# phuang1024/Starst3r

Measured on AMD Instinct MI355X. Metric: 3DGS train iters/sec @ 1M Gaussians, 8x1080p views, higher is better.
Workload: dtype f32

## Files before the change

### include/st3r.h

```cpp
#ifndef ST3R_H
#define ST3R_H

#include <stdint.h>

#ifdef __cplusplus
extern "C" {
#endif

#define ST3R_VERSION 100

#define ST3R_OK 0
#define ST3R_ERR_INVALID (-1)
#define ST3R_ERR_HIP (-2)
#define ST3R_ERR_CAPACITY (-3)
#define ST3R_ERR_NOMEM (-4)
#define ST3R_ERR_PEER (-5)

#define ST3R_SPLAT_STRIDE 12
#define ST3R_MAX_VIEWS 256
#define ST3R_GRAD_PER_GAUSSIAN 23

typedef struct st3r_ctx st3r_ctx;

int st3r_version(void);
// ... 11 lines not shown
int st3r_ctx_release_scratch(st3r_ctx* ctx);
int st3r_ctx_get_stage_ms(st3r_ctx* ctx, double* ms_out, int64_t* counts_out);
const char* st3r_stage_name(int stage);


int st3r_gs_project_sh(st3r_ctx* ctx, void* stream, int N, int C, const float* means, const float* quats,
                       const float* scales, const float* opacities, const float* sh, int sh_stride,
                       const float* viewmats, const float* Ks, const float* campos, int width, int height,
                       int tile_size, float eps2d, float near_plane, float far_plane, float radius_clip,
                       float* splats, int32_t* tiles_per_gauss, double* reg_sums);

int st3r_gs_isect_scan(st3r_ctx* ctx, void* stream, int64_t n_pairs, const int32_t* tiles_per_gauss,
                       int32_t* cum_tiles, int64_t* n_isects_host);

int st3r_gs_isect_emit(st3r_ctx* ctx, void* stream, int N, int C, const float* splats,
                       const int32_t* cum_tiles, int tile_size, int tile_w, int tile_h, int64_t n_isects,
                       int64_t* isect_ids, int32_t* flatten_ids);

int st3r_gs_sort(st3r_ctx* ctx, void* stream, int64_t n_isects, int end_bit, int64_t* isect_ids,
                 int32_t* flatten_ids, int64_t* isect_ids_sorted, int32_t* flatten_ids_sorted);

int st3r_radix_sort_pairs(st3r_ctx* ctx, void* stream, int key_bytes, int64_t n, int begin_bit, int end_bit,
                          const void* keys_in, const int32_t* vals_in, void* keys_out, int32_t* vals_out);

int st3r_gs_offsets(st3r_ctx* ctx, void* stream, int64_t n_isects, const int64_t* isect_ids_sorted, int C,
                    int tile_w, int tile_h, int32_t* offsets);

int st3r_gs_blend_fwd(st3r_ctx* ctx, void* stream, int C, int width, int height, int tile_size, int tile_w,
                      int tile_h, const float* splats, const int32_t* offsets, const int32_t* flatten_ids,
                      int64_t n_isects, float* rgb, float* alpha, int32_t* last_ids);

int st3r_gs_blend_bwd(st3r_ctx* ctx, void* stream, int C, int width, int height, int tile_size, int tile_w,
                      int tile_h, const float* splats, const int32_t* offsets, const int32_t* flatten_ids,
                      int64_t n_isects, const float* alpha, const int32_t* last_ids, const float* v_rgb,
                      const float* v_alpha, const int32_t* cum_tiles, int64_t n_pairs, float* v_splats);

int st3r_gs_project_sh_bwd(st3r_ctx* ctx, void* stream, int N, int C, const float* means, const float* quats,
                           const float* scales, const float* opacities, const float* sh, int sh_stride,
                           const float* viewmats, const float* Ks, const float* campos, int width, int height,
                           float eps2d, const float* splats, const float* v_splats, float reg_views,
                           float opac_fac, float scale_fac, float* grads);

int st3r_gs_viewmat_bwd(st3r_ctx* ctx, void* stream, int N, int C, const float* means, const float* quats,
                        const float* scales, const float* sh, int sh_stride, const float* viewmats, const float* Ks,
                        const float* campos, int width, int height, float eps2d, const float* splats,
                        const float* v_splats, float* v_viewmats);
// ... 141 lines not shown
```

### starst3r_amd/_lib.py

```python
import ctypes as C
import os

_HERE = os.path.dirname(os.path.abspath(__file__))
LIB_PATH = os.path.join(_HERE, "libst3r_hip.so")

_lib = None

vp, i32, i64, f32, f64 = C.c_void_p, C.c_int, C.c_int64, C.c_float, C.c_double
u32, u64 = C.c_uint32, C.c_uint64

SIGNATURES = {
    "st3r_version": [],
    "st3r_last_error": [],
    "st3r_ctx_create": [i32, C.POINTER(vp)],
    "st3r_ctx_destroy": [vp],
    "st3r_ctx_arena_bytes": [vp],
    "st3r_ctx_peek": [vp, vp, i32, vp, i64],
    "st3r_ctx_set_profiling": [vp, i32],
    "st3r_ctx_set_debug": [vp, i32],
    "st3r_ctx_settle": [vp],
    "st3r_ctx_release_scratch": [vp],
    "st3r_ctx_get_stage_ms": [vp, C.POINTER(f64), C.POINTER(i64)],
    "st3r_stage_name": [i32],
    "st3r_gs_project_sh": [vp, vp, i32, i32, vp, vp, vp, vp, vp, i32, vp, vp, vp, i32, i32, i32, f32, f32, f32, f32,
                           vp, vp, vp],
    "st3r_gs_isect_scan": [vp, vp, i64, vp, vp, C.POINTER(i64)],
    "st3r_gs_isect_emit": [vp, vp, i32, i32, vp, vp, i32, i32, i32, i64, vp, vp],
    "st3r_gs_sort": [vp, vp, i64, i32, vp, vp, vp, vp],
    "st3r_radix_sort_pairs": [vp, vp, i32, i64, i32, i32, vp, vp, vp, vp],
    "st3r_gs_offsets": [vp, vp, i64, vp, i32, i32, i32, vp],
    "st3r_gs_blend_fwd": [vp, vp, i32, i32, i32, i32, i32, i32, vp, vp, vp, i64, vp, vp, vp],
    "st3r_gs_blend_bwd": [vp, vp, i32, i32, i32, i32, i32, i32, vp, vp, vp, i64, vp, vp, vp, vp, vp, i64, vp],
    "st3r_gs_project_sh_bwd": [vp, vp, i32, i32, vp, vp, vp, vp, vp, i32, vp, vp, vp, i32, i32, f32, vp, vp, f32, f32,
                               f32, vp],
    "st3r_gs_viewmat_bwd": [vp, vp, i32, i32, vp, vp, vp, vp, i32, vp, vp, vp, i32, i32, f32, vp, vp, vp],
    "st3r_gs_blend_depth_fwd": [vp, vp, i32, i32, i32, i32, i32, i32, vp, vp, vp, i64, vp, vp, vp],
    "st3r_gs_blend_depth_bwd": [vp, vp, i32, i32, i32, i32, i32, i32, vp, vp, vp, i64, vp, vp, vp, vp, i64, vp],
    "st3r_gs_depth_bwd": [vp, vp, i32, i32, vp, vp, vp, vp, vp, vp],
    "st3r_loss_l1_ssim": [vp, vp, i32, i32, i32, vp, vp, f32, f32, vp, vp],
    "st3r_loss_gt_moments": [vp, vp, i32, i32, i32, vp, vp],
    "st3r_ctx_set_gt_moments": [vp, vp, vp, i32, i32, i32],
    "st3r_adam_step": [vp, vp, i32, vp, vp, vp, vp, vp, i32, vp, vp, vp, f64, f64, f64, f64, i32],
    "st3r_adam_step_range": [vp, vp, i32, vp, vp, vp, vp, vp, i32, vp, vp, vp, f64, f64, f64, f64, i32, i64, i64, vp],
    "st3r_params_from_stage": [vp, vp, i32, vp, vp, vp, vp, vp, i32, vp, i64, i64, i64],
    "st3r_gs_train_fwd_bwd": [vp, vp, i32, i32, vp, vp, vp, vp, vp, i32, vp, vp, vp, vp, i32, i32, f32, f32, f32, vp,
                              vp, C.POINTER(i64)],
    "st3r_align_run": [vp, vp, i32, i32, i32, vp, vp, vp, vp, vp, vp, vp, vp, vp, vp, i32, vp, vp, vp, i32, vp, vp,
                       vp, vp, i32, vp, vp, vp, vp, i32, i32, vp, f32, i32, f32, i32, f32, vp, vp, vp, vp, vp, vp, i64,
                       vp, vp, vp],
    "st3r_align_run_opts": [vp, vp, i32, i32, i32, vp, vp, vp, vp, vp, vp, vp, vp, vp, vp, i32, vp, vp, vp, i32, vp, vp,
                            vp, vp, i32, vp, vp, vp, vp, i32, i32, vp, f32, i32, f32, i32, f32, vp, vp, vp, vp, vp, vp,
                            i64, vp, vp, vp, vp, f32, f32, f32, i32, vp, vp, vp, i64],
# ... 66 lines not shown
```

### starst3r_amd/csrc/api.hip

```cpp
#include <stdarg.h>

#include "common.h"

static thread_local char g_err[512] = "";

void st3r_set_error(const char* fmt, ...) {
    va_list ap;
    va_start(ap, fmt);
    vsnprintf(g_err, sizeof(g_err), fmt, ap);
    va_end(ap);
}

ST3R_EXPORT int st3r_version(void) { return ST3R_VERSION; }
ST3R_EXPORT const char* st3r_last_error(void) { return g_err; }

ST3R_EXPORT int st3r_ctx_create(int device, st3r_ctx** out) {
    ARG_CHECK(out);
    int ndev = 0;
    HIP_TRY(hipGetDeviceCount(&ndev));
    ARG_CHECK(device >= 0 && device < ndev);
    HIP_TRY(hipSetDevice(device));
    st3r_ctx* c = new (std::nothrow) st3r_ctx();
    if (!c) { st3r_set_error("out of host memory"); return ST3R_ERR_NOMEM; }
    memset(c, 0, sizeof(*c));
// ... 136 lines not shown
        ctx->prof_ms[st] = 0; ctx->prof_n[st] = 0;
    }
    return ST3R_OK;
}

int st3r_isect_scan_impl(st3r_ctx* ctx, hipStream_t s, int64_t n_pairs, const int32_t* tiles, int32_t* cum,
                         int64_t* n_isects_host, const void* pack_rects, int rect32, uint64_t* pack_out,
                         int32_t** total_dev_out, int32_t* total_copy, int32_t* total_host);
int st3r_isect_emit_impl(hipStream_t s, int N, int C, const float* splats, const int32_t* cum, int tile_size,
                         int tile_w, int tile_h, int64_t* isect_ids, int32_t* flatten_ids);
int st3r_sort_impl(st3r_ctx* ctx, hipStream_t s, int64_t n, int end_bit, int64_t* keys_in, int32_t* vals_in,
                   int64_t* keys_out, int32_t* vals_out);
int st3r_isect_offsets_impl(hipStream_t s, int64_t n_isects, const int64_t* ids, int C, int tile_w, int tile_h,
                            int32_t* offsets);
int st3r_project_impl(st3r_ctx* ctx, hipStream_t s, int N, int C, const float* means, const float* quats, const float* scales,
                      const float* opacities, const float* sh, int sh_stride, const float* viewmats, const float* Ks,
                      const float* campos, int width, int height, int tile_size, float eps2d, float near_plane,
                      float far_plane, float radius_clip, float* splats, int32_t* tiles_per_gauss, double* reg_sums,
                      uint64_t* depth_keys, int32_t* depth_vals, int tight, uint32_t key_base, void* rects, int rect32,
                      int reg_overwrite, double* zero_ptr, int zero_n, uint32_t* krange);
int st3r_sort_depth_seg_impl(st3r_ctx* ctx, hipStream_t s, int64_t N, int C, uint32_t* keys_in, int32_t* vals_in,
                             uint32_t* keys_out, int32_t* vals_out, const uint32_t* krange);
int st3r_isect_emit_chain_impl(st3r_ctx* ctx, hipStream_t s, int N, int C, const int32_t* perm, const void* rects,
                               int rect32, int tile_w, int tile_h, uint32_t* tile_keys, int32_t* vals, int64_t cap);
int st3r_records_prepare_impl(hipStream_t s, int N, int C, const float* splats, int tile_size, int tile_w, int tile_h,
                              int tight, int32_t* tiles, uint64_t* depth_keys, int32_t* depth_vals, uint32_t key_base,
                              void* rects, int rect32);
int st3r_isect_offsets32_impl(hipStream_t s, int64_t n_isects, const uint32_t* keys, int C, int tile_w, int tile_h,
                              int32_t* offsets, const int32_t* n_dev);
int st3r_sort_depth_impl(st3r_ctx* ctx, hipStream_t s, int64_t n, int end_bit, uint64_t* keys_in, int32_t* vals_in,
                         uint64_t* keys_out, int32_t* vals_out);
int st3r_sort_depth32_impl(st3r_ctx* ctx, hipStream_t s, int64_t n, int end_bit, uint32_t* keys_in, int32_t* vals_in,
                           uint32_t* keys_out, int32_t* vals_out);
int st3r_sort_tile_impl(st3r_ctx* ctx, hipStream_t s, int64_t n, int end_bit, uint32_t* keys_in, int32_t* vals_in,
                        uint32_t* keys_out, int32_t* vals_out, const int32_t* n_dev);
int st3r_blend_fwd_impl(st3r_ctx* ctx, hipStream_t s, int C, int W, int H, int tile_w, int tile_h,
                        const float* splats, const int32_t* offsets, const int32_t* flat, int64_t n_isects,
                        float* rgb, float* alpha, int32_t* last_ids, bool for_backward, bool end_in_offsets);
int st3r_blend_bwd_impl(st3r_ctx* ctx, hipStream_t s, int C, int W, int H, int tile_w, int tile_h,
                        const float* splats, const int32_t* offsets, const int32_t* flat, int64_t n_isects,
                        const float* alpha, const int32_t* last_ids, const float* v_rgb, const float* v_alpha,
                        const int32_t* cum, const uint64_t* rects, const uint64_t* rectbase, int tight, int64_t n_pairs,
                        float* v_splats,
                        bool end_in_offsets, st3r_vtile_ref* defer);
int st3r_project_sh_bwd_impl(hipStream_t s, int N, int C, const float* means, const float* quats, const float* scales,
                             const float* opacities, const float* sh, int sh_stride, const float* viewmats,
                             const float* Ks, const float* campos, int width, int height, float eps2d,
                             const float* splats, const float* v_splats, float reg_views, float opac_fac,
                             float scale_fac, float* grads, bool accumulate, int g_begin, int g_end, bool range_major,
                             const st3r_vtile_ref* slots);
int st3r_loss_impl(st3r_ctx* ctx, hipStream_t s, int C, int H, int W, const float* render, const float* gt,
                   float w_l1, float w_ssim, double* sums, float* v_render, bool sums_cleared);
int st3r_gather_vtile_impl(hipStream_t s, int64_t n_pairs, const st3r_vtile_ref* slots, float* v_splats);

static int bit_length_u32(uint32_t v) { int n = 0; while (v) { ++n; v >>= 1; } return n; }

static int settle_pending_count(st3r_ctx* ctx) {
    if (!ctx->count_pending) return ST3R_OK;
// ... 127 lines not shown
    st3r_prof_end(ctx, s, STG_SCAN);
    if (rc) return rc;
    if (async) {
        if (!ctx->count_event) HIP_TRY(hipEventCreateWithFlags(&ctx->count_event, hipEventDisableTiming));
        HIP_TRY(hipEventRecord(ctx->count_event, s));
        n_isects = ctx->isect_hint + ctx->isect_hint / 4 + 1024;
        if (ctx->debug_flags & 8) n_isects = ctx->isect_hint / 2;
        if (n_isects > 2147483647LL) n_isects = 2147483647LL;
        ctx->count_pending = 1; ctx->count_cap = n_isects;
        o->n_visible = -1; o->n_isects_ref = -1;
    } else {
        HIP_TRY(hipMemcpyAsync(ctx->pinned, total_dev, sizeof(int32_t), hipMemcpyDeviceToHost, s));
        if (reg_sums) HIP_TRY(hipMemcpyAsync(ctx->pinned + 1, reg_sums + 2, 2 * sizeof(double), hipMemcpyDeviceToHost, s));
        HIP_TRY(hipStreamSynchronize(s));
        n_isects = (int64_t)((int32_t*)ctx->pinned)[0];
        if (n_isects < 0) {
            st3r_set_error("more than 2^31 tile intersections in one call: split the views over more calls / GPUs");
            return ST3R_SPLIT_VIEWS;
        }
        o->n_visible = reg_sums ? (int64_t)((double*)ctx->pinned)[1] : -1;
        o->n_isects_ref = reg_sums ? (int64_t)((double*)ctx->pinned)[2] : n_isects;
        if (allow_async) { ctx->isect_hint = n_isects; ctx->hint_sig = sig; }
    }
    GET(SLOT_KEYS_A, uint32_t, n_isects, tkeys_a);
    GET(SLOT_KEYS_B, uint32_t, n_isects, tkeys_b);
    GET(SLOT_VALS_A, int32_t, n_isects, vals_a);
    GET(SLOT_VALS_B, int32_t, n_isects, vals_b);
    n_dev = total_dev;
    o->n_records = async ? -1 : n_isects;
    if (n_isects > 0) {
        st3r_prof_begin(ctx, s, STG_EMIT);
        rc = st3r_isect_emit_chain_impl(ctx, s, N, C, perm, rects, rect32, tile_w, tile_h, tkeys_a, vals_a, n_isects);
        st3r_prof_end(ctx, s, STG_EMIT);
        if (rc) return rc;
        const int end_bit = bit_length_u32((uint32_t)((int64_t)C * tile_w * tile_h - 1));
        st3r_prof_begin(ctx, s, STG_SORT);
        rc = st3r_sort_tile_impl(ctx, s, n_isects, end_bit, tkeys_a, vals_a, tkeys_b, vals_b, n_dev);
        st3r_prof_end(ctx, s, STG_SORT);
        if (rc) return rc;
    }
    st3r_prof_begin(ctx, s, STG_OFFSETS);
    rc = st3r_isect_offsets32_impl(s, n_isects, tkeys_b, C, tile_w, tile_h, offsets, n_dev);
    st3r_prof_end(ctx, s, STG_OFFSETS);
    if (rc) return rc;
    o->splats = splats; o->offsets = offsets; o->flat = vals_b; o->cum = cum; o->rects = rect32 ? nullptr : rects;
    o->rectbase = rectbase;
    o->n_isects = n_isects;
    o->tile_w = tile_w; o->tile_h = tile_h;
    return ST3R_OK;
}

__global__ void k_finalize_loss(int C, const double* __restrict__ sums, const double* __restrict__ reg_sums,
                                double inv_px, double inv_cnt, double w_l1, double w_ssim, double reg_views,
                                double opac_k, double scale_k, float* __restrict__ loss_out) {
    if (threadIdx.x == 0 && blockIdx.x == 0) {
        double loss = 0;
        for (int c = 0; c < C; ++c) loss += w_l1 * sums[2 * c] * inv_px + w_ssim * (1.0 - sums[2 * c + 1] * inv_cnt);
        loss += reg_views * (opac_k * reg_sums[0] + scale_k * reg_sums[1]);
        loss_out[0] = (float)loss;
    }
}

static int train_views(st3r_ctx* ctx, hipStream_t s, int N, int C, const float* means, const float* quats,
                       const float* scales, const float* opacities, const float* sh, int sh_stride,
                       const float* viewmats, const float* Ks, const float* campos, const float* gt_images, int W, int H,
// ... 204 lines not shown
```

### starst3r_amd/csrc/gs_isect.hip

```cpp
#include "common.h"
#include "tile_rect.h"

#define SCAN_THREADS 256
#define SCAN_ITEMS 16
#define SCAN_TILE (SCAN_THREADS * SCAN_ITEMS)

__device__ __forceinline__ int wave_incl_scan(int v) {
    const int lane = threadIdx.x & 63;
#pragma unroll
    for (int off = 1; off < 64; off <<= 1) {
        int t = __shfl_up(v, off);
        if (lane >= off) v += t;
    }
    return v;
}

__device__ __forceinline__ int block_incl_scan(int v, int* total) {
    __shared__ int wsum[4];
    const int lane = threadIdx.x & 63, w = threadIdx.x >> 6;
    int inc = wave_incl_scan(v);
    if (lane == 63) wsum[w] = inc;
    __syncthreads();
    int base = 0;
#pragma unroll
// ... 255 lines not shown
}

int st3r_isect_offsets_impl(hipStream_t s, int64_t n_isects, const int64_t* ids, int C, int tile_w, int tile_h,
                            int32_t* offsets) {
    int n_tiles = tile_w * tile_h;
    if (n_isects == 0) {
        HIP_TRY(hipMemsetAsync(offsets, 0, sizeof(int32_t) * (size_t)C * n_tiles, s));
        return ST3R_OK;
    }
    int tile_n_bits = bit_length_u32((uint32_t)n_tiles);
    hipLaunchKernelGGL(k_isect_offsets, dim3(ceil_div(n_isects, 256)), dim3(256), 0, s, n_isects, ids, C, n_tiles,
                       tile_n_bits, offsets);
    LAUNCH_CHECK();
    return ST3R_OK;
}

ST3R_EXPORT int st3r_gs_offsets(st3r_ctx* ctx, void* stream, int64_t n_isects, const int64_t* isect_ids_sorted,
                                int C, int tile_w, int tile_h, int32_t* offsets) {
    ARG_CHECK(ctx && n_isects >= 0 && C > 0 && tile_w > 0 && tile_h > 0 && offsets);
    ARG_CHECK(n_isects == 0 || isect_ids_sorted);
    return st3r_isect_offsets_impl((hipStream_t)stream, n_isects, isect_ids_sorted, C, tile_w, tile_h, offsets);
}

__global__ __launch_bounds__(256) void k_isect_offsets32(int64_t n_isects, const uint32_t* __restrict__ keys,
                                                         int64_t total, int32_t* __restrict__ offsets,
                                                         const int32_t* __restrict__ n_dev) {
    if (n_dev) n_isects = min(n_isects, (int64_t)max(*n_dev, 0));
    const int64_t tid = (int64_t)blockIdx.x * blockDim.x + threadIdx.x;
    if (n_isects == 0) {
        for (int64_t i = tid; i <= total; i += (int64_t)gridDim.x * blockDim.x) offsets[i] = 0;
        return;
    }
    const int64_t i0 = tid * 4;
    if (i0 >= n_isects) return;
    uint32_t k[4];
    if (i0 + 4 <= n_isects) {
        const uint4 v = *reinterpret_cast<const uint4*>(keys + i0);
        k[0] = v.x; k[1] = v.y; k[2] = v.z; k[3] = v.w;
    } else {
#pragma unroll
        for (int j = 0; j < 4; ++j) k[j] = i0 + j < n_isects ? keys[i0 + j] : 0u;
    }
    int64_t prev = i0 == 0 ? -1 : (int64_t)keys[i0 - 1];
#pragma unroll
    for (int j = 0; j < 4; ++j) {
        const int64_t idx = i0 + j;
        if (idx < n_isects) {
            const int64_t cur = k[j];
            for (int64_t i = prev + 1; i <= cur; ++i) offsets[i] = (int32_t)idx;
            prev = cur;
            if (idx == n_isects - 1)
                for (int64_t i = cur + 1; i <= total; ++i) offsets[i] = (int32_t)n_isects;
        }
    }
}

int st3r_isect_offsets32_impl(hipStream_t s, int64_t n_isects, const uint32_t* keys, int C, int tile_w, int tile_h,
                              int32_t* offsets, const int32_t* n_dev) {
    const int64_t total = (int64_t)C * tile_w * tile_h;
    if (n_isects == 0 && !n_dev) {
        HIP_TRY(hipMemsetAsync(offsets, 0, sizeof(int32_t) * (size_t)(total + 1), s));
        return ST3R_OK;
    }
    hipLaunchKernelGGL(k_isect_offsets32, dim3(ceil_div(n_isects > 0 ? (n_isects + 3) / 4 : 1, 256)), dim3(256), 0, s, n_isects,
                       keys, total, offsets, n_dev);
    LAUNCH_CHECK();
    return ST3R_OK;
}

__global__ __launch_bounds__(256) void k_records_prepare(int N, int64_t n_pairs, const float4* __restrict__ splats,
                                                         int tile_size, int tile_w, int tile_h, int tight,
                                                         int32_t* __restrict__ tiles, uint64_t* __restrict__ depth_keys,
                                                         int32_t* __restrict__ depth_vals, uint32_t key_base,
                                                         void* __restrict__ rects, int rect32) {
    const int64_t pid = (int64_t)blockIdx.x * blockDim.x + threadIdx.x;
    if (pid >= n_pairs) return;
    const float4 r2 = splats[pid * 3 + 2];
    const int radius = __float_as_int(r2.z);
    int ntiles = 0;
    TileRect tr = {0, 0, 0, 0};
    if (radius > 0) {
        const float4 r0 = splats[pid * 3 + 0];
        tr = ref_tile_rect(r0.x, r0.y, (float)radius, tile_size, tile_w, tile_h);
        if (tight) {
            const float4 r1 = splats[pid * 3 + 1];
            tr = tight_tile_rect(tr, r0.x, r0.y, r0.z, r0.w, r1.x, r1.y);
        }
        ntiles = (tr.y1 - tr.y0) * (tr.x1 - tr.x0);
// ... 70 lines not shown
__global__ __launch_bounds__(1024) void k_isect_wg_scan(int n, const int32_t* __restrict__ wg_tiles,
                                                        long long* __restrict__ wg_base) {
    __shared__ long long s_wave[16];
    const int t = threadIdx.x, lane = t & 63, w = t >> 6;
    const int per = (n + 1023) / 1024;
    const int e0 = min(t * per, n), e1 = min(e0 + per, n);
    long long sum = 0;
    for (int e = e0; e < e1; ++e) sum += wg_tiles[e];
    long long inc = sum;
#pragma unroll
    for (int off = 1; off < 64; off <<= 1) {
        const long long o = __shfl_up(inc, off);
        if (lane >= off) inc += o;
    }
    if (lane == 63) s_wave[w] = inc;
    __syncthreads();
    long long base = 0;
#pragma unroll
    for (int i = 0; i < 16; ++i) base += i < w ? s_wave[i] : 0;
    long long run = base + inc - sum;
    for (int e = e0; e < e1; ++e) { wg_base[e] = run; run += wg_tiles[e]; }
}

__global__ __launch_bounds__(256) void k_isect_emit_d(int N, int C, int bpc, const int32_t* __restrict__ perm,
                                                      const void* __restrict__ rects_d, int rect32,
                                                      const long long* __restrict__ wg_base,
                                                      const int32_t* __restrict__ wg_tiles, int tile_w, int tile_h,
                                                      uint32_t* __restrict__ tile_keys, int32_t* __restrict__ vals,
                                                      int64_t cap) {
    __shared__ int s_end[EP];
    __shared__ uint32_t s_org[EP];
    __shared__ uint16_t s_w[EP];
    __shared__ int32_t s_pid[EP];
    __shared__ uint16_t s_own[ECH];
    __shared__ unsigned s_wmax[4];
    __shared__ long long s_bsum[4];
    int c, k;
    emit_item(C, bpc, &c, &k);
    const int t = threadIdx.x, lane = t & 63, w = t >> 6;
    long long bsum = 0;
    if (!wg_base) {
        const int nb4 = (c * bpc + k) >> 2;
        for (int i = t; i < nb4; i += 256) {
            const int4 v = reinterpret_cast<const int4*>(wg_tiles)[i];
            bsum += ((long long)v.x + v.y) + ((long long)v.z + v.w);
        }
        if (t < ((c * bpc + k) & 3)) bsum += wg_tiles[4 * nb4 + t];
    }
    const int64_t first = (int64_t)c * N + (int64_t)k * EP;
    const int np = (int)min((int64_t)EP, (int64_t)(c + 1) * N - first);
    int cnt[EPT];
// ... 68 lines not shown
            if (ww < w) pre = max(pre, s_wmax[ww]);
        carry_owner = (int)max(max(max((unsigned)carry_owner, s_wmax[0]), max(s_wmax[1], s_wmax[2])), s_wmax[3]);
#pragma unroll
        for (int i = 0; i < 8; ++i) {
            const unsigned lo = max(wv[i] & 0xFFFFu, pre), hi = max(wv[i] >> 16, pre);
            wv[i] = lo | (hi << 16);
        }
        reinterpret_cast<uint4*>(s_own)[2 * t] = make_uint4(wv[0], wv[1], wv[2], wv[3]);
        reinterpret_cast<uint4*>(s_own)[2 * t + 1] = make_uint4(wv[4], wv[5], wv[6], wv[7]);
        __syncthreads();
        const int lim = min(ECH, total - c0);
        for (int i = t; i < lim; i += 256) {
            const int p = (int)s_own[i] - 1;
            const int o = c0 + i;
            const int kk = o - (p == 0 ? 0 : s_end[p - 1]);
            const uint32_t w_ = s_w[p], org = s_org[p];
            int qq = (int)((float)kk * __builtin_amdgcn_rcpf((float)w_));
            int rem = kk - qq * (int)w_;
            if (rem < 0) { --qq; rem += (int)w_; }
            if (rem >= (int)w_) { ++qq; rem -= (int)w_; }
            const uint32_t tx = (org & 0xFFFF) + (uint32_t)rem, ty = (org >> 16) + (uint32_t)qq;
            const long long pos = base + o;
            if (pos >= 0 && pos < cap) {
                tile_keys[pos] = key0 + ty * (uint32_t)tile_w + tx;
                vals[pos] = s_pid[p];
            }
        }
        __syncthreads();
    }
}

int st3r_isect_emit_chain_impl(st3r_ctx* ctx, hipStream_t s, int N, int C, const int32_t* perm, const void* rects,
                               int rect32, int tile_w, int tile_h, uint32_t* tile_keys, int32_t* vals, int64_t cap) {
    const int64_t n_pairs = (int64_t)N * C;
    if (n_pairs == 0) return ST3R_OK;
    const int bpc = ceil_div(N, EP);
    const int grid = C * bpc;
    void* p;
    int rc = st3r_arena_get(ctx, SLOT_RECTS_D, (rect32 ? sizeof(uint32_t) : sizeof(uint64_t)) * (size_t)n_pairs, &p);
    if (rc) return rc;
    void* rects_d = p;
    rc = st3r_arena_get(ctx, SLOT_CUM_D, (sizeof(long long) + sizeof(int32_t)) * (size_t)grid + 16, &p);
    if (rc) return rc;
    long long* wg_base = (long long*)p;
    int32_t* wg_tiles = (int32_t*)(wg_base + grid);
    if (((uintptr_t)wg_tiles & 15) != 0) wg_tiles += 2;
    hipLaunchKernelGGL(k_isect_gather, dim3(grid), dim3(256), 0, s, N, C, bpc, perm, rects, rect32, rects_d, wg_tiles);
    const bool self_base = grid <= EMIT_SELF_BASE_MAX;
    if (!self_base) hipLaunchKernelGGL(k_isect_wg_scan, dim3(1), dim3(1024), 0, s, grid, wg_tiles, wg_base);
    hipLaunchKernelGGL(k_isect_emit_d, dim3(grid), dim3(256), 0, s, N, C, bpc, perm, rects_d, rect32,
                       self_base ? (const long long*)nullptr : wg_base, wg_tiles, tile_w, tile_h, tile_keys, vals, cap);
    LAUNCH_CHECK();
    return ST3R_OK;
}
```

### starst3r_amd/csrc/gs_sort.hip

```cpp
#include "common.h"
#include "radix_sort.h"

int st3r_sort_impl(st3r_ctx* ctx, hipStream_t s, int64_t n, int end_bit, int64_t* keys_in, int32_t* vals_in,
                   int64_t* keys_out, int32_t* vals_out) {
    if (end_bit > 64) end_bit = 64;
    return st3r_radix_sort_u64(ctx, s, n, 0, end_bit, reinterpret_cast<const uint64_t*>(keys_in), vals_in,
                               reinterpret_cast<uint64_t*>(keys_out), vals_out);
}

int st3r_sort_depth_impl(st3r_ctx* ctx, hipStream_t s, int64_t n, int end_bit, uint64_t* keys_in, int32_t* vals_in,
                         uint64_t* keys_out, int32_t* vals_out) {
    return st3r_radix_sort_u64(ctx, s, n, 0, end_bit, keys_in, vals_in, keys_out, vals_out);
}

int st3r_sort_depth32_impl(st3r_ctx* ctx, hipStream_t s, int64_t n, int end_bit, uint32_t* keys_in, int32_t* vals_in,
                           uint32_t* keys_out, int32_t* vals_out) {
    return st3r_radix_sort_u32(ctx, s, n, 0, end_bit, keys_in, vals_in, keys_out, vals_out);
}

int st3r_sort_depth_seg_impl(st3r_ctx* ctx, hipStream_t s, int64_t N, int C, uint32_t* keys_in, int32_t* vals_in,
                             uint32_t* keys_out, int32_t* vals_out, const uint32_t* krange) {
    return st3r_radix_sort_u32_segments(ctx, s, N, C, keys_in, vals_in, keys_out, vals_out, krange);
}

int st3r_sort_tile_impl(st3r_ctx* ctx, hipStream_t s, int64_t n, int end_bit, uint32_t* keys_in, int32_t* vals_in,
                        uint32_t* keys_out, int32_t* vals_out, const int32_t* n_dev) {
    if (n_dev) return st3r_radix_sort_u32_devcount(ctx, s, n, n_dev, 0, end_bit, keys_in, vals_in, keys_out, vals_out);
    return st3r_radix_sort_u32(ctx, s, n, 0, end_bit, keys_in, vals_in, keys_out, vals_out);
}

ST3R_EXPORT int st3r_gs_sort(st3r_ctx* ctx, void* stream, int64_t n_isects, int end_bit, int64_t* isect_ids,
                             int32_t* flatten_ids, int64_t* isect_ids_sorted, int32_t* flatten_ids_sorted) {
    ARG_CHECK(ctx && n_isects >= 0 && end_bit > 0);
    if (n_isects == 0) return ST3R_OK;
    ARG_CHECK(isect_ids && flatten_ids && isect_ids_sorted && flatten_ids_sorted);
    return st3r_sort_impl(ctx, (hipStream_t)stream, n_isects, end_bit, isect_ids, flatten_ids, isect_ids_sorted,
                          flatten_ids_sorted);
}

ST3R_EXPORT int st3r_radix_sort_pairs(st3r_ctx* ctx, void* stream, int key_bytes, int64_t n, int begin_bit, int end_bit,
                                      const void* keys_in, const int32_t* vals_in, void* keys_out, int32_t* vals_out) {
    ARG_CHECK(ctx && n >= 0 && (key_bytes == 4 || key_bytes == 8) && begin_bit >= 0 && end_bit > begin_bit);
    ARG_CHECK(end_bit <= 8 * key_bytes && n < 2147483647LL);
    if (n == 0) return ST3R_OK;
    ARG_CHECK(keys_in && keys_out && ((vals_in == nullptr) == (vals_out == nullptr)));
    if (key_bytes == 4)
        return st3r_radix_sort_u32(ctx, (hipStream_t)stream, n, begin_bit, end_bit, (const uint32_t*)keys_in, vals_in,
                                   (uint32_t*)keys_out, vals_out);
    return st3r_radix_sort_u64(ctx, (hipStream_t)stream, n, begin_bit, end_bit, (const uint64_t*)keys_in, vals_in,
                               (uint64_t*)keys_out, vals_out);
}
```

### starst3r_amd/csrc/radix_sort.h

```cpp
#pragma once
#include "common.h"

int st3r_radix_sort_u32(st3r_ctx* ctx, hipStream_t s, int64_t n, int begin_bit, int end_bit, const uint32_t* keys_in,
                        const int32_t* vals_in, uint32_t* keys_out, int32_t* vals_out);
int st3r_radix_sort_u64(st3r_ctx* ctx, hipStream_t s, int64_t n, int begin_bit, int end_bit, const uint64_t* keys_in,
                        const int32_t* vals_in, uint64_t* keys_out, int32_t* vals_out);
int st3r_radix_sort_u32_devcount(st3r_ctx* ctx, hipStream_t s, int64_t n_cap, const int32_t* n_dev, int begin_bit,
                                 int end_bit, const uint32_t* keys_in, const int32_t* vals_in, uint32_t* keys_out,
                                 int32_t* vals_out);
int st3r_radix_sort_u32_segments(st3r_ctx* ctx, hipStream_t s, int64_t seg_n, int n_seg, const uint32_t* keys_in,
                                 const int32_t* vals_in, uint32_t* keys_out, int32_t* vals_out, const uint32_t* krange);
```

### starst3r_amd/csrc/radix_sort.hip

```cpp
#include "radix_sort.h"

namespace {

constexpr int RB = 8;
constexpr int RADIX = 1 << RB;
#ifndef RS_THREADS
#define RS_THREADS 1024
#endif
#ifndef RS_SMALL_BELOW
#define RS_SMALL_BELOW 100
#endif
constexpr int THREADS_L = RS_THREADS, THREADS_S = 512;
constexpr int HIST_THREADS = 256;
constexpr int HIST_ITEMS = 16;
constexpr int MAX_PASSES = 8;
constexpr int HIST_COPIES = 8;

typedef unsigned long long u64;
constexpr u64 FLAG_AGG = 1ull << 62, FLAG_INC = 2ull << 62, VALUE_MASK = (1ull << 62) - 1;

template <typename K> struct Traits;
#ifndef RS_IPT32
#define RS_IPT32 16
#endif
template <> struct Traits<uint32_t> { static constexpr int IPT = RS_IPT32, IPT_S = 8; };
template <> struct Traits<uint64_t> { static constexpr int IPT = 8, IPT_S = 4; };

__device__ __forceinline__ int wave_incl_scan_u32(uint32_t v, int lane) {
#pragma unroll
    for (int off = 1; off < 64; off <<= 1) {
        const uint32_t t = __shfl_up(v, off);
        if (lane >= off) v += t;
    }
    return v;
}

__device__ __forceinline__ uint32_t pair_lane_u32(uint32_t v, int q) {
    return q == 0 ? (uint32_t)__builtin_amdgcn_mov_dpp((int)v, 0xA0, 0xf, 0xf, true)
                  : (uint32_t)__builtin_amdgcn_mov_dpp((int)v, 0xF5, 0xf, 0xf, true);
}
__device__ __forceinline__ uint32_t quad_lane_u32(uint32_t v, int q) {
    switch (q) {
        case 0: return (uint32_t)__builtin_amdgcn_mov_dpp((int)v, 0x00, 0xf, 0xf, true);
        case 1: return (uint32_t)__builtin_amdgcn_mov_dpp((int)v, 0x55, 0xf, 0xf, true);
        case 2: return (uint32_t)__builtin_amdgcn_mov_dpp((int)v, 0xAA, 0xf, 0xf, true);
        default: return (uint32_t)__builtin_amdgcn_mov_dpp((int)v, 0xFF, 0xf, 0xf, true);
    }
}

template <typename K>
__global__ __launch_bounds__(HIST_THREADS) void k_rs_hist(const K* __restrict__ keys, int64_t n, int begin_bit,
                                                          int end_bit, int passes, uint32_t* __restrict__ hist,
                                                          const int32_t* __restrict__ n_dev) {
    __shared__ uint32_t sh[HIST_THREADS / 64][MAX_PASSES * RADIX];
    if (n_dev) n = min(n, (int64_t)max(*n_dev, 0));
    for (int i = threadIdx.x; i < (HIST_THREADS / 64) * MAX_PASSES * RADIX; i += HIST_THREADS) (&sh[0][0])[i] = 0;
    __syncthreads();
    uint32_t* mine = sh[threadIdx.x >> 6];
    constexpr int CH = HIST_THREADS * HIST_ITEMS;
    for (int64_t base = (int64_t)blockIdx.x * CH; base < n; base += (int64_t)gridDim.x * CH) {
        K k[HIST_ITEMS];
#pragma unroll
        for (int i = 0; i < HIST_ITEMS; ++i) {
            const int64_t idx = base + i * HIST_THREADS + threadIdx.x;
            k[i] = idx < n ? keys[idx] : K(0);
        }
#pragma unroll
        for (int i = 0; i < HIST_ITEMS; ++i) {
            if (base + i * HIST_THREADS + threadIdx.x < n) {
                for (int p = 0; p < passes; ++p) {
                    const int shift = begin_bit + RB * p;
                    const int bits = min(RB, end_bit - shift);
                    atomicAdd(&mine[p * RADIX + ((uint32_t)(k[i] >> shift) & ((1u << bits) - 1u))], 1u);
                }
            }
        }
    }
    __syncthreads();
    for (int i = threadIdx.x; i < passes * RADIX; i += HIST_THREADS) {
        uint32_t t = 0;
#pragma unroll
        for (int w = 0; w < HIST_THREADS / 64; ++w) t += sh[w][i];
// ... 224 lines not shown
    __syncthreads();
#pragma unroll
    for (int i = 0; i < IPT; ++i) {
        const int p = i * THREADS + tid;
        if (p < tcount) {
            const K k = sbuf[p];
            const uint32_t d = (uint32_t)(k >> shift) & dmask;
            const long long o = gofs[d] + p;
            if (!(SEG && last_seg_pass)) kout[o] = k;
            if (has_vals) vout[o] = svals[p];
        }
    }
}

inline size_t align256(size_t v) { return (v + 255) & ~(size_t)255; }

template <typename K>
int sort_pairs(st3r_ctx* ctx, hipStream_t s, int64_t n, int begin_bit, int end_bit, const K* keys_in,
               const int32_t* vals_in, K* keys_out, int32_t* vals_out, const int32_t* n_dev = nullptr) {
    if (n == 0) return ST3R_OK;
    if (end_bit > (int)sizeof(K) * 8) end_bit = (int)sizeof(K) * 8;
    if (begin_bit < 0 || begin_bit >= end_bit) { st3r_set_error("radix sort: empty bit range"); return ST3R_ERR_INVALID; }
    const int passes = (end_bit - begin_bit + RB - 1) / RB;
    constexpr int TILE_L = THREADS_L * Traits<K>::IPT, TILE_S = THREADS_S * Traits<K>::IPT_S;
    const bool small = (n + TILE_L - 1) / TILE_L < RS_SMALL_BELOW;
    const int64_t TILE = small ? TILE_S : TILE_L;
    const int64_t ntiles = (n + TILE - 1) / TILE;
    const size_t hist_bytes = align256(sizeof(uint32_t) * (size_t)(HIST_COPIES * MAX_PASSES * RADIX + MAX_PASSES));
    const size_t status_bytes = sizeof(u64) * (size_t)passes * (size_t)ntiles * RADIX;
    const size_t meta_bytes = hist_bytes + align256(status_bytes);
    const bool need_tmp = passes > 1;
    const size_t tk_bytes = need_tmp ? align256(sizeof(K) * (size_t)n) : 0;
    const size_t tv_bytes = need_tmp && vals_in ? align256(sizeof(int32_t) * (size_t)n) : 0;
    void* p;
    int rc = st3r_arena_get(ctx, SLOT_SORT_TMP, meta_bytes + tk_bytes + tv_bytes, &p);
    if (rc) return rc;
    char* base = (char*)p;
    uint32_t* hist = (uint32_t*)base;
    uint32_t* counters = hist + HIST_COPIES * MAX_PASSES * RADIX;
    u64* status = (u64*)(base + hist_bytes);
    K* tk = (K*)(base + meta_bytes);
    int32_t* tv = (int32_t*)(base + meta_bytes + tk_bytes);
    HIP_TRY(hipMemsetAsync(base, 0, meta_bytes, s));
    const int hist_blocks = (int)min((int64_t)1024, (n + HIST_THREADS * HIST_ITEMS - 1) / (HIST_THREADS * HIST_ITEMS));
    hipLaunchKernelGGL(k_rs_hist<K>, dim3(hist_blocks), dim3(HIST_THREADS), 0, s, keys_in, n, begin_bit, end_bit, passes,
                       hist, n_dev);
    const K* kin = keys_in;
    const int32_t* vin = vals_in;
    for (int ps = 0; ps < passes; ++ps) {
        const bool to_out = ((passes - 1 - ps) & 1) == 0;
        K* ko = to_out ? keys_out : tk;
        int32_t* vo = to_out ? vals_out : tv;
        const int shift = begin_bit + RB * ps;
        const int bits = min(RB, end_bit - shift);
        if (small)
            hipLaunchKernelGGL((k_rs_pass<K, THREADS_S, Traits<K>::IPT_S>), dim3((unsigned)ntiles), dim3(THREADS_S), 0, s, kin,
                               vin, ko, vin ? vo : nullptr, n, shift, bits, hist + ps * RADIX,
                               status + (size_t)ps * ntiles * RADIX, counters + ps, n_dev);
        else
            hipLaunchKernelGGL((k_rs_pass<K, THREADS_L, Traits<K>::IPT>), dim3((unsigned)ntiles), dim3(THREADS_L), 0, s, kin,
                               vin, ko, vin ? vo : nullptr, n, shift, bits, hist + ps * RADIX,
                               status + (size_t)ps * ntiles * RADIX, counters + ps, n_dev);
        kin = ko;
        if (vin) vin = vo;
    }
    LAUNCH_CHECK();
    return ST3R_OK;
}

// ... 42 lines not shown

}

int st3r_radix_sort_u32_segments(st3r_ctx* ctx, hipStream_t s, int64_t seg_n, int n_seg, const uint32_t* keys_in,
                                 const int32_t* vals_in, uint32_t* keys_out, int32_t* vals_out, const uint32_t* krange) {
    return sort_pairs_seg(ctx, s, seg_n, n_seg, keys_in, vals_in, keys_out, vals_out, krange);
}

int st3r_radix_sort_u32(st3r_ctx* ctx, hipStream_t s, int64_t n, int begin_bit, int end_bit, const uint32_t* keys_in,
                        const int32_t* vals_in, uint32_t* keys_out, int32_t* vals_out) {
    return sort_pairs<uint32_t>(ctx, s, n, begin_bit, end_bit, keys_in, vals_in, keys_out, vals_out);
}

int st3r_radix_sort_u64(st3r_ctx* ctx, hipStream_t s, int64_t n, int begin_bit, int end_bit, const uint64_t* keys_in,
                        const int32_t* vals_in, uint64_t* keys_out, int32_t* vals_out) {
    return sort_pairs<uint64_t>(ctx, s, n, begin_bit, end_bit, keys_in, vals_in, keys_out, vals_out);
}

int st3r_radix_sort_u32_devcount(st3r_ctx* ctx, hipStream_t s, int64_t n_cap, const int32_t* n_dev, int begin_bit,
                                 int end_bit, const uint32_t* keys_in, const int32_t* vals_in, uint32_t* keys_out,
                                 int32_t* vals_out) {
    return sort_pairs<uint32_t>(ctx, s, n_cap, begin_bit, end_bit, keys_in, vals_in, keys_out, vals_out, n_dev);
}
```

### starst3r_amd/ops.py

```python
import ctypes as C
import math

import torch

from . import _lib

SPLAT = 12
TILE = 16


class Context:

    def __init__(self, device):
        self.device = torch.device(device)
        if self.device.type != "cuda":
            raise _lib.St3rError(f"the st3r hot path needs a GPU device, got {device!r} (no CPU fallback)")
        idx = self.device.index if self.device.index is not None else torch.cuda.current_device()
        self.device = torch.device("cuda", idx)
        self._h = C.c_void_p()
        with torch.cuda.device(idx):
            _lib.check(_lib.lib().st3r_ctx_create(idx, C.byref(self._h)))
        import os
        if os.environ.get("ST3R_DEBUG_FLAGS"):
            _lib.check(_lib.lib().st3r_ctx_set_debug(self._h, int(os.environ["ST3R_DEBUG_FLAGS"])))
# ... 91 lines not shown

def isect(ctx, splats, tiles, N, Cn, W, H):
    tw, th = tile_grid(W, H)
    cum = torch.empty_like(tiles)
    n = C.c_int64(0)
    _lib.check(_lib.lib().st3r_gs_isect_scan(ctx.handle, _stream(), N * Cn, _p(tiles, torch.int32),
                                             _p(cum, torch.int32), C.byref(n)))
    n = n.value
    ids = torch.empty((n,), dtype=torch.int64, device=splats.device)
    flat = torch.empty((n,), dtype=torch.int32, device=splats.device)
    _lib.check(_lib.lib().st3r_gs_isect_emit(ctx.handle, _stream(), N, Cn, _p(splats), _p(cum, torch.int32), TILE, tw,
                                             th, n, _p(ids, torch.int64), _p(flat, torch.int32)))
    return cum, ids, flat


def radix_sort_pairs(ctx, keys, vals, begin_bit, end_bit):
    assert keys.dtype in (torch.int32, torch.int64)
    kb = 4 if keys.dtype == torch.int32 else 8
    ko = torch.empty_like(keys)
    vo = torch.empty_like(vals) if vals is not None else None
    _lib.check(_lib.lib().st3r_radix_sort_pairs(ctx.handle, _stream(), kb, keys.numel(), begin_bit, end_bit,
                                                _p(keys, keys.dtype), _p(vals, torch.int32), _p(ko, keys.dtype),
                                                _p(vo, torch.int32)))
    return ko, vo


def sort_pairs(ctx, ids, flat, end_bit):
    ids_in, flat_in = ids.clone(), flat.clone()
    ids_out, flat_out = torch.empty_like(ids), torch.empty_like(flat)
    _lib.check(_lib.lib().st3r_gs_sort(ctx.handle, _stream(), ids.numel(), end_bit, _p(ids_in, torch.int64),
                                       _p(flat_in, torch.int32), _p(ids_out, torch.int64),
                                       _p(flat_out, torch.int32)))
    return ids_out, flat_out


def offsets(ctx, ids_sorted, Cn, W, H):
    tw, th = tile_grid(W, H)
    off = torch.empty((Cn, th, tw), dtype=torch.int32, device=ids_sorted.device)
    _lib.check(_lib.lib().st3r_gs_offsets(ctx.handle, _stream(), ids_sorted.numel(), _p(ids_sorted, torch.int64), Cn,
                                          tw, th, _p(off, torch.int32)))
    return off


def blend_fwd(ctx, splats, off, flat, Cn, W, H):
    tw, th = tile_grid(W, H)
    dev = splats.device
# ... 359 lines not shown
```

Before: 190.7.

## Use 16-bit tile keys for intersection emit, sort and offsets when they fit

When the total tile count across views fits in 16 bits, tile keys are stored as uint16. The emit, radix sort (including a paired histogram read) and offsets kernels are templated on key width to work with them. This halves key memory traffic and arena footprint in the sort pipeline. It adds template instantiations, a new exported u16 sort, and a fallback to 32-bit keys via a debug flag or when the tile count is large.

```diff
diff --git a/include/st3r.h b/include/st3r.h
--- a/include/st3r.h
+++ b/include/st3r.h
@@ -57,6 +57,9 @@
 
 int st3r_radix_sort_pairs(st3r_ctx* ctx, void* stream, int key_bytes, int64_t n, int begin_bit, int end_bit,
                           const void* keys_in, const int32_t* vals_in, void* keys_out, int32_t* vals_out);
+
+int st3r_radix_sort_u16(st3r_ctx* ctx, void* stream, int64_t n, int begin_bit, int end_bit, const uint16_t* keys_in,
+                        const int32_t* vals_in, uint16_t* keys_out, int32_t* vals_out);
 
 int st3r_gs_offsets(st3r_ctx* ctx, void* stream, int64_t n_isects, const int64_t* isect_ids_sorted, int C,
                     int tile_w, int tile_h, int32_t* offsets);
diff --git a/starst3r_amd/_lib.py b/starst3r_amd/_lib.py
--- a/starst3r_amd/_lib.py
+++ b/starst3r_amd/_lib.py
@@ -28,6 +28,7 @@
     "st3r_gs_isect_emit": [vp, vp, i32, i32, vp, vp, i32, i32, i32, i64, vp, vp],
     "st3r_gs_sort": [vp, vp, i64, i32, vp, vp, vp, vp],
     "st3r_radix_sort_pairs": [vp, vp, i32, i64, i32, i32, vp, vp, vp, vp],
+    "st3r_radix_sort_u16": [vp, vp, i64, i32, i32, vp, vp, vp, vp],
     "st3r_gs_offsets": [vp, vp, i64, vp, i32, i32, i32, vp],
     "st3r_gs_blend_fwd": [vp, vp, i32, i32, i32, i32, i32, i32, vp, vp, vp, i64, vp, vp, vp],
     "st3r_gs_blend_bwd": [vp, vp, i32, i32, i32, i32, i32, i32, vp, vp, vp, i64, vp, vp, vp, vp, vp, i64, vp],
diff --git a/starst3r_amd/csrc/api.hip b/starst3r_amd/csrc/api.hip
--- a/starst3r_amd/csrc/api.hip
+++ b/starst3r_amd/csrc/api.hip
@@ -182,18 +182,19 @@
 int st3r_sort_depth_seg_impl(st3r_ctx* ctx, hipStream_t s, int64_t N, int C, uint32_t* keys_in, int32_t* vals_in,
                              uint32_t* keys_out, int32_t* vals_out, const uint32_t* krange);
 int st3r_isect_emit_chain_impl(st3r_ctx* ctx, hipStream_t s, int N, int C, const int32_t* perm, const void* rects,
-                               int rect32, int tile_w, int tile_h, uint32_t* tile_keys, int32_t* vals, int64_t cap);
+                               int rect32, int tile_w, int tile_h, void* tile_keys, int key16, int32_t* vals,
+                               int64_t cap);
 int st3r_records_prepare_impl(hipStream_t s, int N, int C, const float* splats, int tile_size, int tile_w, int tile_h,
                               int tight, int32_t* tiles, uint64_t* depth_keys, int32_t* depth_vals, uint32_t key_base,
                               void* rects, int rect32);
-int st3r_isect_offsets32_impl(hipStream_t s, int64_t n_isects, const uint32_t* keys, int C, int tile_w, int tile_h,
+int st3r_isect_offsets32_impl(hipStream_t s, int64_t n_isects, const void* keys, int key16, int C, int tile_w, int tile_h,
                               int32_t* offsets, const int32_t* n_dev);
 int st3r_sort_depth_impl(st3r_ctx* ctx, hipStream_t s, int64_t n, int end_bit, uint64_t* keys_in, int32_t* vals_in,
                          uint64_t* keys_out, int32_t* vals_out);
 int st3r_sort_depth32_impl(st3r_ctx* ctx, hipStream_t s, int64_t n, int end_bit, uint32_t* keys_in, int32_t* vals_in,
                            uint32_t* keys_out, int32_t* vals_out);
-int st3r_sort_tile_impl(st3r_ctx* ctx, hipStream_t s, int64_t n, int end_bit, uint32_t* keys_in, int32_t* vals_in,
-                        uint32_t* keys_out, int32_t* vals_out, const int32_t* n_dev);
+int st3r_sort_tile_impl(st3r_ctx* ctx, hipStream_t s, int64_t n, int end_bit, void* keys_in, int32_t* vals_in,
+                        void* keys_out, int32_t* vals_out, const int32_t* n_dev, int key16);
 int st3r_blend_fwd_impl(st3r_ctx* ctx, hipStream_t s, int C, int W, int H, int tile_w, int tile_h,
                         const float* splats, const int32_t* offsets, const int32_t* flat, int64_t n_isects,
                         float* rgb, float* alpha, int32_t* last_ids, bool for_backward, bool end_in_offsets);
@@ -367,25 +368,31 @@
         o->n_isects_ref = reg_sums ? (int64_t)((double*)ctx->pinned)[2] : n_isects;
         if (allow_async) { ctx->isect_hint = n_isects; ctx->hint_sig = sig; }
     }
-    GET(SLOT_KEYS_A, uint32_t, n_isects, tkeys_a);
-    GET(SLOT_KEYS_B, uint32_t, n_isects, tkeys_b);
+    const int end_bit = bit_length_u32((uint32_t)((int64_t)C * tile_w * tile_h - 1));
+    const int key16 = (end_bit <= 16 && !(ctx->debug_flags & 256)) ? 1 : 0;
+    void *tkeys_a, *tkeys_b;
+    {
+        const size_t kb = (key16 ? sizeof(uint16_t) : sizeof(uint32_t)) * (size_t)n_isects;
+        int rc_ = st3r_arena_get(ctx, SLOT_KEYS_A, kb, &tkeys_a);
+        if (!rc_) rc_ = st3r_arena_get(ctx, SLOT_KEYS_B, kb, &tkeys_b);
+        if (rc_) return rc_;
+    }
     GET(SLOT_VALS_A, int32_t, n_isects, vals_a);
     GET(SLOT_VALS_B, int32_t, n_isects, vals_b);
     n_dev = total_dev;
     o->n_records = async ? -1 : n_isects;
     if (n_isects > 0) {
         st3r_prof_begin(ctx, s, STG_EMIT);
-        rc = st3r_isect_emit_chain_impl(ctx, s, N, C, perm, rects, rect32, tile_w, tile_h, tkeys_a, vals_a, n_isects);
+        rc = st3r_isect_emit_chain_impl(ctx, s, N, C, perm, rects, rect32, tile_w, tile_h, tkeys_a, key16, vals_a, n_isects);
         st3r_prof_end(ctx, s, STG_EMIT);
         if (rc) return rc;
-        const int end_bit = bit_length_u32((uint32_t)((int64_t)C * tile_w * tile_h - 1));
         st3r_prof_begin(ctx, s, STG_SORT);
-        rc = st3r_sort_tile_impl(ctx, s, n_isects, end_bit, tkeys_a, vals_a, tkeys_b, vals_b, n_dev);
+        rc = st3r_sort_tile_impl(ctx, s, n_isects, end_bit, tkeys_a, vals_a, tkeys_b, vals_b, n_dev, key16);
         st3r_prof_end(ctx, s, STG_SORT);
         if (rc) return rc;
     }
     st3r_prof_begin(ctx, s, STG_OFFSETS);
-    rc = st3r_isect_offsets32_impl(s, n_isects, tkeys_b, C, tile_w, tile_h, offsets, n_dev);
+    rc = st3r_isect_offsets32_impl(s, n_isects, tkeys_b, key16, C, tile_w, tile_h, offsets, n_dev);
     st3r_prof_end(ctx, s, STG_OFFSETS);
     if (rc) return rc;
     o->splats = splats; o->offsets = offsets; o->flat = vals_b; o->cum = cum; o->rects = rect32 ? nullptr : rects;
diff --git a/starst3r_amd/csrc/gs_isect.hip b/starst3r_amd/csrc/gs_isect.hip
--- a/starst3r_amd/csrc/gs_isect.hip
+++ b/starst3r_amd/csrc/gs_isect.hip
@@ -301,7 +301,8 @@
     return st3r_isect_offsets_impl((hipStream_t)stream, n_isects, isect_ids_sorted, C, tile_w, tile_h, offsets);
 }
 
-__global__ __launch_bounds__(256) void k_isect_offsets32(int64_t n_isects, const uint32_t* __restrict__ keys,
+template <typename K>
+__global__ __launch_bounds__(256) void k_isect_offsets32(int64_t n_isects, const K* __restrict__ keys,
                                                          int64_t total, int32_t* __restrict__ offsets,
                                                          const int32_t* __restrict__ n_dev) {
     if (n_dev) n_isects = min(n_isects, (int64_t)max(*n_dev, 0));
@@ -314,8 +315,13 @@
     if (i0 >= n_isects) return;
     uint32_t k[4];
     if (i0 + 4 <= n_isects) {
-        const uint4 v = *reinterpret_cast<const uint4*>(keys + i0);
-        k[0] = v.x; k[1] = v.y; k[2] = v.z; k[3] = v.w;
+        if constexpr (sizeof(K) == 4) {
+            const uint4 v = *reinterpret_cast<const uint4*>(keys + i0);
+            k[0] = v.x; k[1] = v.y; k[2] = v.z; k[3] = v.w;
+        } else {
+            const uint2 v = *reinterpret_cast<const uint2*>(keys + i0);
+            k[0] = v.x & 0xFFFFu; k[1] = v.x >> 16; k[2] = v.y & 0xFFFFu; k[3] = v.y >> 16;
+        }
     } else {
 #pragma unroll
         for (int j = 0; j < 4; ++j) k[j] = i0 + j < n_isects ? keys[i0 + j] : 0u;
@@ -334,15 +340,20 @@
     }
 }
 
-int st3r_isect_offsets32_impl(hipStream_t s, int64_t n_isects, const uint32_t* keys, int C, int tile_w, int tile_h,
+int st3r_isect_offsets32_impl(hipStream_t s, int64_t n_isects, const void* keys, int key16, int C, int tile_w, int tile_h,
                               int32_t* offsets, const int32_t* n_dev) {
     const int64_t total = (int64_t)C * tile_w * tile_h;
     if (n_isects == 0 && !n_dev) {
         HIP_TRY(hipMemsetAsync(offsets, 0, sizeof(int32_t) * (size_t)(total + 1), s));
         return ST3R_OK;
     }
-    hipLaunchKernelGGL(k_isect_offsets32, dim3(ceil_div(n_isects > 0 ? (n_isects + 3) / 4 : 1, 256)), dim3(256), 0, s, n_isects,
-                       keys, total, offsets, n_dev);
+    const dim3 grid(ceil_div(n_isects > 0 ? (n_isects + 3) / 4 : 1, 256));
+    if (key16)
+        hipLaunchKernelGGL(k_isect_offsets32<uint16_t>, grid, dim3(256), 0, s, n_isects, (const uint16_t*)keys, total, offsets,
+                           n_dev);
+    else
+        hipLaunchKernelGGL(k_isect_offsets32<uint32_t>, grid, dim3(256), 0, s, n_isects, (const uint32_t*)keys, total, offsets,
+                           n_dev);
     LAUNCH_CHECK();
     return ST3R_OK;
 }
@@ -459,11 +470,12 @@
     for (int e = e0; e < e1; ++e) { wg_base[e] = run; run += wg_tiles[e]; }
 }
 
+template <typename K>
 __global__ __launch_bounds__(256) void k_isect_emit_d(int N, int C, int bpc, const int32_t* __restrict__ perm,
                                                       const void* __restrict__ rects_d, int rect32,
                                                       const long long* __restrict__ wg_base,
                                                       const int32_t* __restrict__ wg_tiles, int tile_w, int tile_h,
-                                                      uint32_t* __restrict__ tile_keys, int32_t* __restrict__ vals,
+                                                      K* __restrict__ tile_keys, int32_t* __restrict__ vals,
                                                       int64_t cap) {
     __shared__ int s_end[EP];
     __shared__ uint32_t s_org[EP];
@@ -578,7 +590,7 @@
             const uint32_t tx = (org & 0xFFFF) + (uint32_t)rem, ty = (org >> 16) + (uint32_t)qq;
             const long long pos = base + o;
             if (pos >= 0 && pos < cap) {
-                tile_keys[pos] = key0 + ty * (uint32_t)tile_w + tx;
+                tile_keys[pos] = (K)(key0 + ty * (uint32_t)tile_w + tx);
                 vals[pos] = s_pid[p];
             }
         }
@@ -587,7 +599,8 @@
 }
 
 int st3r_isect_emit_chain_impl(st3r_ctx* ctx, hipStream_t s, int N, int C, const int32_t* perm, const void* rects,
-                               int rect32, int tile_w, int tile_h, uint32_t* tile_keys, int32_t* vals, int64_t cap) {
+                               int rect32, int tile_w, int tile_h, void* tile_keys, int key16, int32_t* vals,
+                               int64_t cap) {
     const int64_t n_pairs = (int64_t)N * C;
     if (n_pairs == 0) return ST3R_OK;
     const int bpc = ceil_div(N, EP);
@@ -604,8 +617,13 @@
     hipLaunchKernelGGL(k_isect_gather, dim3(grid), dim3(256), 0, s, N, C, bpc, perm, rects, rect32, rects_d, wg_tiles);
     const bool self_base = grid <= EMIT_SELF_BASE_MAX;
     if (!self_base) hipLaunchKernelGGL(k_isect_wg_scan, dim3(1), dim3(1024), 0, s, grid, wg_tiles, wg_base);
-    hipLaunchKernelGGL(k_isect_emit_d, dim3(grid), dim3(256), 0, s, N, C, bpc, perm, rects_d, rect32,
-                       self_base ? (const long long*)nullptr : wg_base, wg_tiles, tile_w, tile_h, tile_keys, vals, cap);
+    const long long* base_arg = self_base ? (const long long*)nullptr : wg_base;
+    if (key16)
+        hipLaunchKernelGGL(k_isect_emit_d<uint16_t>, dim3(grid), dim3(256), 0, s, N, C, bpc, perm, rects_d, rect32, base_arg,
+                           wg_tiles, tile_w, tile_h, (uint16_t*)tile_keys, vals, cap);
+    else
+        hipLaunchKernelGGL(k_isect_emit_d<uint32_t>, dim3(grid), dim3(256), 0, s, N, C, bpc, perm, rects_d, rect32, base_arg,
+                           wg_tiles, tile_w, tile_h, (uint32_t*)tile_keys, vals, cap);
     LAUNCH_CHECK();
     return ST3R_OK;
 }
diff --git a/starst3r_amd/csrc/gs_sort.hip b/starst3r_amd/csrc/gs_sort.hip
--- a/starst3r_amd/csrc/gs_sort.hip
+++ b/starst3r_amd/csrc/gs_sort.hip
@@ -23,8 +23,13 @@
     return st3r_radix_sort_u32_segments(ctx, s, N, C, keys_in, vals_in, keys_out, vals_out, krange);
 }
 
-int st3r_sort_tile_impl(st3r_ctx* ctx, hipStream_t s, int64_t n, int end_bit, uint32_t* keys_in, int32_t* vals_in,
-                        uint32_t* keys_out, int32_t* vals_out, const int32_t* n_dev) {
+int st3r_sort_tile_impl(st3r_ctx* ctx, hipStream_t s, int64_t n, int end_bit, void* keys_in_, int32_t* vals_in,
+                        void* keys_out_, int32_t* vals_out, const int32_t* n_dev, int key16) {
+    if (key16)
+        return st3r_radix_sort_u16_devcount(ctx, s, n, n_dev, 0, end_bit, (const uint16_t*)keys_in_, vals_in,
+                                            (uint16_t*)keys_out_, vals_out);
+    uint32_t* keys_in = (uint32_t*)keys_in_;
+    uint32_t* keys_out = (uint32_t*)keys_out_;
     if (n_dev) return st3r_radix_sort_u32_devcount(ctx, s, n, n_dev, 0, end_bit, keys_in, vals_in, keys_out, vals_out);
     return st3r_radix_sort_u32(ctx, s, n, 0, end_bit, keys_in, vals_in, keys_out, vals_out);
 }
@@ -50,3 +55,13 @@
     return st3r_radix_sort_u64(ctx, (hipStream_t)stream, n, begin_bit, end_bit, (const uint64_t*)keys_in, vals_in,
                                (uint64_t*)keys_out, vals_out);
 }
+
+ST3R_EXPORT int st3r_radix_sort_u16(st3r_ctx* ctx, void* stream, int64_t n, int begin_bit, int end_bit,
+                                    const uint16_t* keys_in, const int32_t* vals_in, uint16_t* keys_out,
+                                    int32_t* vals_out) {
+    ARG_CHECK(ctx && n >= 0 && begin_bit >= 0 && end_bit > begin_bit && end_bit <= 16 && n < 2147483647LL);
+    if (n == 0) return ST3R_OK;
+    ARG_CHECK(keys_in && keys_out && ((vals_in == nullptr) == (vals_out == nullptr)));
+    return st3r_radix_sort_u16_devcount(ctx, (hipStream_t)stream, n, nullptr, begin_bit, end_bit, keys_in, vals_in,
+                                        keys_out, vals_out);
+}
diff --git a/starst3r_amd/csrc/radix_sort.h b/starst3r_amd/csrc/radix_sort.h
--- a/starst3r_amd/csrc/radix_sort.h
+++ b/starst3r_amd/csrc/radix_sort.h
@@ -8,5 +8,8 @@
 int st3r_radix_sort_u32_devcount(st3r_ctx* ctx, hipStream_t s, int64_t n_cap, const int32_t* n_dev, int begin_bit,
                                  int end_bit, const uint32_t* keys_in, const int32_t* vals_in, uint32_t* keys_out,
                                  int32_t* vals_out);
+int st3r_radix_sort_u16_devcount(st3r_ctx* ctx, hipStream_t s, int64_t n_cap, const int32_t* n_dev, int begin_bit,
+                                 int end_bit, const uint16_t* keys_in, const int32_t* vals_in, uint16_t* keys_out,
+                                 int32_t* vals_out);
 int st3r_radix_sort_u32_segments(st3r_ctx* ctx, hipStream_t s, int64_t seg_n, int n_seg, const uint32_t* keys_in,
                                  const int32_t* vals_in, uint32_t* keys_out, int32_t* vals_out, const uint32_t* krange);
diff --git a/starst3r_amd/csrc/radix_sort.hip b/starst3r_amd/csrc/radix_sort.hip
--- a/starst3r_amd/csrc/radix_sort.hip
+++ b/starst3r_amd/csrc/radix_sort.hip
@@ -23,8 +23,12 @@
 #ifndef RS_IPT32
 #define RS_IPT32 16
 #endif
-template <> struct Traits<uint32_t> { static constexpr int IPT = RS_IPT32, IPT_S = 8; };
-template <> struct Traits<uint64_t> { static constexpr int IPT = 8, IPT_S = 4; };
+#ifndef RS_THREADS16
+#define RS_THREADS16 RS_THREADS
+#endif
+template <> struct Traits<uint16_t> { static constexpr int IPT = 16, IPT_S = 8, THREADS_L = RS_THREADS16; };
+template <> struct Traits<uint32_t> { static constexpr int IPT = RS_IPT32, IPT_S = 8, THREADS_L = RS_THREADS; };
+template <> struct Traits<uint64_t> { static constexpr int IPT = 8, IPT_S = 4, THREADS_L = RS_THREADS; };
 
 __device__ __forceinline__ int wave_incl_scan_u32(uint32_t v, int lane) {
 #pragma unroll
@@ -51,13 +55,43 @@
 template <typename K>
 __global__ __launch_bounds__(HIST_THREADS) void k_rs_hist(const K* __restrict__ keys, int64_t n, int begin_bit,
                                                           int end_bit, int passes, uint32_t* __restrict__ hist,
-                                                          const int32_t* __restrict__ n_dev) {
+                                                          const int32_t* __restrict__ n_dev, int pairs) {
     __shared__ uint32_t sh[HIST_THREADS / 64][MAX_PASSES * RADIX];
     if (n_dev) n = min(n, (int64_t)max(*n_dev, 0));
     for (int i = threadIdx.x; i < (HIST_THREADS / 64) * MAX_PASSES * RADIX; i += HIST_THREADS) (&sh[0][0])[i] = 0;
     __syncthreads();
     uint32_t* mine = sh[threadIdx.x >> 6];
     constexpr int CH = HIST_THREADS * HIST_ITEMS;
+    if constexpr (sizeof(K) == 2) {
+        if (pairs) {
+            const uint32_t* kw = reinterpret_cast<const uint32_t*>(keys);
+            const int64_t nw = (n + 1) >> 1;
+            for (int64_t base = (int64_t)blockIdx.x * CH; base < nw; base += (int64_t)gridDim.x * CH) {
+                uint32_t k[HIST_ITEMS];
+#pragma unroll
+                for (int i = 0; i < HIST_ITEMS; ++i) {
+                    const int64_t idx = base + i * HIST_THREADS + threadIdx.x;
+                    k[i] = 2 * idx + 1 < n ? kw[idx] : (2 * idx < n ? (uint32_t)keys[2 * idx] : 0u);
+                }
+#pragma unroll
+                for (int i = 0; i < HIST_ITEMS; ++i) {
+                    const int64_t idx = base + i * HIST_THREADS + threadIdx.x;
+#pragma unroll
+                    for (int h = 0; h < 2; ++h) {
+                        if (2 * idx + h < n) {
+                            const uint32_t kk = h ? k[i] >> 16 : k[i] & 0xFFFFu;
+                            for (int p = 0; p < passes; ++p) {
+                                const int shift = begin_bit + RB * p;
+                                const int bits = min(RB, end_bit - shift);
+                                atomicAdd(&mine[p * RADIX + ((kk >> shift) & ((1u << bits) - 1u))], 1u);
+                            }
+                        }
+                    }
+                }
+            }
+            n = 0;
+        }
+    }
     for (int64_t base = (int64_t)blockIdx.x * CH; base < n; base += (int64_t)gridDim.x * CH) {
         K k[HIST_ITEMS];
 #pragma unroll
@@ -328,6 +362,7 @@
     if (end_bit > (int)sizeof(K) * 8) end_bit = (int)sizeof(K) * 8;
     if (begin_bit < 0 || begin_bit >= end_bit) { st3r_set_error("radix sort: empty bit range"); return ST3R_ERR_INVALID; }
     const int passes = (end_bit - begin_bit + RB - 1) / RB;
+    constexpr int THREADS_L = Traits<K>::THREADS_L;
     constexpr int TILE_L = THREADS_L * Traits<K>::IPT, TILE_S = THREADS_S * Traits<K>::IPT_S;
     const bool small = (n + TILE_L - 1) / TILE_L < RS_SMALL_BELOW;
     const int64_t TILE = small ? TILE_S : TILE_L;
@@ -348,9 +383,11 @@
     K* tk = (K*)(base + meta_bytes);
     int32_t* tv = (int32_t*)(base + meta_bytes + tk_bytes);
     HIP_TRY(hipMemsetAsync(base, 0, meta_bytes, s));
-    const int hist_blocks = (int)min((int64_t)1024, (n + HIST_THREADS * HIST_ITEMS - 1) / (HIST_THREADS * HIST_ITEMS));
+    const int hist_pairs = sizeof(K) == 2 && ((uintptr_t)keys_in & 3) == 0 ? 1 : 0;
+    const int64_t hist_chunk = (int64_t)HIST_THREADS * HIST_ITEMS * (hist_pairs ? 2 : 1);
+    const int hist_blocks = (int)min((int64_t)1024, (n + hist_chunk - 1) / hist_chunk);
     hipLaunchKernelGGL(k_rs_hist<K>, dim3(hist_blocks), dim3(HIST_THREADS), 0, s, keys_in, n, begin_bit, end_bit, passes,
-                       hist, n_dev);
+                       hist, n_dev, hist_pairs);
     const K* kin = keys_in;
     const int32_t* vin = vals_in;
     for (int ps = 0; ps < passes; ++ps) {
@@ -439,3 +476,9 @@
                                  int32_t* vals_out) {
     return sort_pairs<uint32_t>(ctx, s, n_cap, begin_bit, end_bit, keys_in, vals_in, keys_out, vals_out, n_dev);
 }
+
+int st3r_radix_sort_u16_devcount(st3r_ctx* ctx, hipStream_t s, int64_t n_cap, const int32_t* n_dev, int begin_bit,
+                                 int end_bit, const uint16_t* keys_in, const int32_t* vals_in, uint16_t* keys_out,
+                                 int32_t* vals_out) {
+    return sort_pairs<uint16_t>(ctx, s, n_cap, begin_bit, end_bit, keys_in, vals_in, keys_out, vals_out, n_dev);
+}
diff --git a/starst3r_amd/ops.py b/starst3r_amd/ops.py
--- a/starst3r_amd/ops.py
+++ b/starst3r_amd/ops.py
@@ -137,6 +137,15 @@
     _lib.check(_lib.lib().st3r_radix_sort_pairs(ctx.handle, _stream(), kb, keys.numel(), begin_bit, end_bit,
                                                 _p(keys, keys.dtype), _p(vals, torch.int32), _p(ko, keys.dtype),
                                                 _p(vo, torch.int32)))
+    return ko, vo
+
+
+def radix_sort_u16(ctx, keys, vals, begin_bit, end_bit):
+    ko = torch.empty_like(keys)
+    vo = torch.empty_like(vals) if vals is not None else None
+    _lib.check(_lib.lib().st3r_radix_sort_u16(ctx.handle, _stream(), keys.numel(), begin_bit, end_bit,
+                                              _p(keys, torch.int16), _p(vals, torch.int32), _p(ko, torch.int16),
+                                              _p(vo, torch.int32)))
     return ko, vo
 
 
```

Result: no change. 190.0, median of 4 (-0.4%).
